# akamiru/bce

Measured on AMD Instinct MI355X. Metric: MB/s compressed, higher is better.
Workload: dtype u8/u32 integer

## Files before the change

### bce_amd/csrc/api.hip

```cpp
#include <condition_variable>
#include <functional>
#include <mutex>
#include <thread>
#include <new>
#include <utility>

#include "bce_cost.h"
#include "common.h"
#include "host_coder.h"
#include "scan_coder.h"

#include <dlfcn.h>
#include <errno.h>
#include <fcntl.h>
#include <sys/file.h>
#include <sys/mman.h>
#include <sys/stat.h>
#include <unistd.h>

using namespace bce;

#ifndef K3_BATCH_MID
#define K3_BATCH_MID 8u
#endif
// ... 336 lines not shown
  bool wide_once = false;
  int dfs_try = 0;
  const uint32_t dfs_enter[2];
  FlushPredictor predict;
  uint32_t round_limit = kNoLimit;
  bool paused = false;

  Enumeration(bce_hip_ctx *ctx, std::function<int(uint64_t)> to)
      : c(ctx), sink(std::move(to)), env(ctx), n(ctx->n), dfs_enter{env.dfs_enter, 2048u} {
    for (int i = 0; i < 8; ++i) { const uint32_t Ci = c->zeros[(i + 7) & 7]; cur_nodes += (Ci && n - Ci) ? 1 : 0; }
  }
  bool finished() const { return ctl.done_round != 0xFFFFFFFFu; }
  int flush() { BCE_TRY(sink(ctl.sym_total)); ctl.sym_total = 0; return BCE_HIP_OK; }
  int grow_lists() { BCE_TRY(k3_grow_lists(c, ctl)); ctl.overflow = 0; return BCE_HIP_OK; }
  int clock_start() { BCE_HIP_TRY(c, hipEventRecord(c->ev0, c->stream)); return BCE_HIP_OK; }
  int clock_stop(bool read_ctl) {
    BCE_HIP_TRY(c, hipEventRecord(c->ev1, c->stream));
    if (read_ctl) BCE_TRY(k3_sync_ctl(c, &ctl));
    else BCE_HIP_TRY(c, hipEventSynchronize(c->ev1));
    float ms = 0;
    if (hipEventElapsedTime(&ms, c->ev0, c->ev1) == hipSuccess) c->stats.k3_ms += ms;
    return BCE_HIP_OK;
  }

  int run() {
    paused = false;
    for (Next next = Next::kRounds; next != Next::kFinished && next != Next::kPaused;) {
      BCE_TRY(gate_regain(c));
      next = Next::kRounds;
      BCE_TRY(pause(&next));
      if (next == Next::kRounds) BCE_TRY(depth_first(&next));
      if (next == Next::kRounds) BCE_TRY(batch(&next));
    }
// ... 46 lines not shown
      while (cut < b.rounds && est < want) { est += nn; nn *= 2; ++cut; }
      b.rounds = cut ? cut : 1u;
    }
    if (!env.no_predict && have_ctl && !ctl.need_flush) b.rounds = predict.rounds_that_fit(b.rounds, c->sym_cap, ctl.sym_total, decaying);
    return b;
  }
  int run_batch(const Batch &b) {
    const uint32_t first = c->round;
    RoctxRange range("bce K3 rounds");
    BCE_TRY(clock_start());
    switch (b.how) {
      case Kernels::kTail: BCE_TRY(k3_tail(c, b.rounds)); break;
      case Kernels::kSmall: BCE_TRY(k3_rounds_small(c, b.rounds, b.nodes, b.growing)); break;
      case Kernels::kWide: BCE_TRY(k3_rounds(c, b.rounds, b.nodes)); break;
    }
    BCE_TRY(clock_stop(true));
    if (ctl.stalled) return k3_stalled(c);
    uint32_t executed = ctl.tail_rounds;
    if (b.how == Kernels::kTail) {
      BCE_TRY(k3_fetch_tail_runs(c, executed));
    } else {
      const bool stopped = ctl.need_flush || ctl.overflow || (b.how == Kernels::kSmall && ctl.small_bail);
      executed = stopped ? ctl.skip_round - first : b.rounds;
      if (executed > b.rounds) return k3_bad_skip(c, ctl, first, b.rounds);
      BCE_TRY(k3_fetch_runs(c, first, executed));
      if (executed) predict.record(reinterpret_cast<const RunEntry *>(c->h_runs), executed, decaying);
    }
    c->round = first + executed;
    return BCE_HIP_OK;
  }
  int batch(Next *next) {
    const Batch b = plan();
    if (!b.rounds) return flush();
    BCE_TRY(run_batch(b));
    if (b.how == Kernels::kSmall && ctl.small_bail) { BCE_TRY(k3_clear_small_bail(c)); wide_once = true; }
    if (ctl.overflow) {
      BCE_TRY(grow_lists());
      have_ctl = true; cur_nodes = 0;
      for (int p = 0; p < 8; ++p) cur_nodes += (uint64_t)ctl.cnt[c->round & 1u][p][0] + ctl.cnt[c->round & 1u][p][1];
      *next = Next::kSameRound;
// ... 124 lines not shown
  (void)hipSetDevice(c->device);
  if (c->coder) c->coder->drain();
  if (c->stream) (void)hipStreamSynchronize(c->stream);
  if (c->k4_stream) (void)hipStreamSynchronize(c->k4_stream);
  if (c->copy_stream) (void)hipStreamSynchronize(c->copy_stream);
  DevBuf *bufs[] = {&c->text, &c->bwt, &c->sa[0], &c->sa[1], &c->key[0], &c->key[1], &c->rank, &c->k2, &c->nrk, &c->act[0], &c->act[1], &c->khi[0], &c->khi[1], &c->dl[0], &c->dl[1], &c->dl[2], &c->dl[3], &c->kflag, &c->actv[0], &c->actv[1],
                    &c->rs_hist, &c->blk, &c->ptmp[0], &c->ptmp[1], &c->gran, &c->nlist[0], &c->nlist[1], &c->ctl, &c->tilecnt,
                    &c->tileoff, &c->runs, &c->smwords, &c->k3tw, &c->k3grp, &c->truns, &c->skey[0], &c->skey[1], &c->sval[0], &c->sval[1], &c->sout,
                    &c->sesc, &c->stat, &c->crc_tab, &c->dcfg, &c->k4w, &c->scanrec, &c->dfs, &c->skey_alt, &c->sesc_alt, &c->rs_hist_k4, &c->cost_acc, &c->cost_runs, &c->cmp_res, &c->hook[0], &c->hook[1], &c->hook[2]};
  for (DevBuf *b : bufs) release(*b);
  for (DevBuf &b : c->qbuf) release(b);
  for (auto &par : c->dlist) for (DevBuf &b : par) release(b);
  k4_prepin_join(c, true);
  if (c->h_ctl) (void)hipHostFree(c->h_ctl);
  if (c->h_small) (void)hipHostFree(c->h_small);
  if (c->h_big) big_host_free(c, c->h_big, c->h_big_cap, c->h_big_registered);
  for (void *q : c->dec_pin) if (q) (void)hipHostFree(q);
  if (c->h_runs) (void)hipHostFree(c->h_runs);
  if (c->h_truns) (void)hipHostFree(c->h_truns);
  if (c->coder) c->coder->drain();
  for (FlushSlot &sl : c->slot) {
    slot_free_host(sl, &c->reg_unmaps);
    if (sl.ev_start) (void)hipEventDestroy(sl.ev_start);
    if (sl.ev_copy) (void)hipEventDestroy(sl.ev_copy);
    if (sl.ev_kend) (void)hipEventDestroy(sl.ev_kend);
    if (sl.h_cost_runs) (void)hipHostFree(sl.h_cost_runs);
  }
  if (c->ev_k4) (void)hipEventDestroy(c->ev_k4);
  if (c->ev_k3_batch) (void)hipEventDestroy(c->ev_k3_batch);
  for (hipEvent_t e : c->ev_k4_done) if (e) (void)hipEventDestroy(e);
// ... 282 lines not shown
  if (c->stat.cap < need || c->dcfg.cap < sizeof(PlaneCfg) * 8) return BCE_HIP_E_STATE;
  BCE_HIP_TRY(c, hipMemcpyAsync(c->dcfg.p, c->cfg, sizeof(PlaneCfg) * 8, hipMemcpyHostToDevice, c->stream));
  BCE_TRY(ensure(c, c->skey[0], (size_t)count * 4));
  BCE_TRY(ensure(c, c->sesc, (size_t)count * 4));
  BCE_HIP_TRY(c, hipMemcpyAsync(c->skey[0].p, key_words, (size_t)count * 4, hipMemcpyHostToDevice, c->stream));
  BCE_HIP_TRY(c, hipMemcpyAsync(c->sesc.p, esc_words, (size_t)count * 4, hipMemcpyHostToDevice, c->stream));
  BCE_HIP_TRY(c, hipStreamSynchronize(c->stream));
  BCE_TRY(k4_flush(c, count, c->slot[0]));
  memcpy(out_records, c->slot[0].h_out, (size_t)count * 8);
  uint32_t nq = 0;
  BCE_TRY(k4_long_runs(c, count, &nq));
  if (long_runs) *long_runs = nq;
  return BCE_HIP_OK;
}

static int encode_start(bce_hip_ctx *c) {
  c->gate_wait_s = 0; c->gate_held_s = 0; c->gate_lent = false;
  gate_acquire(c);
  BCE_HIP_TRY(c, hipSetDevice(c->device));
  const uint32_t n = c->n;
  k4_prepin(c, n);
  BCE_TRY(k4_prepare(c));
  BCE_TRY(k3_begin(c));
  uint32_t C[8];
  for (int i = 0; i < 8; ++i) C[i] = c->zeros[(i + 7) & 7];
  c->coder->begin(c->config, C, n);
  memset(c->plane_syms, 0, sizeof c->plane_syms);
  c->stats.symbols = 0; c->stats.flushes = 0; c->stats.t_model = 0; c->stats.t_model_kernels = 0; c->stats.t_coder = 0;
  return BCE_HIP_OK;
}
static int encode_end(bce_hip_ctx *c, const EnumCtl &ctl, double t_enc0) {
  gate_release(c);
  c->gate_lent = false;
  static const bool gate_timing = getenv("BCE_HIP_GATE_TIMING") != nullptr;
  const double t_gpu_done = now_s();
  {
    const double tw = now_s();
    c->coder->drain();
    c->stats.t_coder += now_s() - tw;
    for (FlushSlot &sl : c->slot) account_slot(c, sl);
  }
  if (c->coder->failed()) { snprintf(c->err, sizeof c->err, "host allocation failed in a range-coder thread"); return BCE_HIP_E_NOMEM; }
  c->stats.t_coder_busy = c->coder->busy_seconds();
// ... 4 lines not shown
  c->stage = 4;
  c->stats.t_enum = c->stats.k3_ms * 1e-3;
  if (gate_timing)
    fprintf(stderr, "gate: ctx %p waited %.1f ms, held %.1f ms of %.1f ms from encode's start to its last flush queued (K3 %.1f ms, model %.1f ms, %llu flushes); coders' tail %.1f ms\n",
            (void *)c, c->gate_wait_s * 1e3, c->gate_held_s * 1e3, (t_gpu_done - t_enc0) * 1e3, c->stats.k3_ms, c->stats.t_model * 1e3,
            (unsigned long long)c->stats.flushes, (now_s() - t_gpu_done) * 1e3);
  return BCE_HIP_OK;
}

static int encode_body(bce_hip_ctx *c);
int bce_hip_encode(bce_hip_ctx *c) { return gate_on_error(c, bce_guarded(c, [&] { return encode_body(c); })); }
static int encode_body(bce_hip_ctx *c) {
  BCE_TRY(check_stage(c, 3));
  PhaseScope phase(c, 3);
  const double t_enc0 = now_s();
  BCE_TRY(encode_start(c));
  Enumeration e(c, [&](uint64_t nsym) { return flush_symbols(c, nsym); });
  BCE_TRY(e.run());
  return encode_end(c, e.ctl, t_enc0);
}

static bool early_enum_applies(const bce_hip_ctx *c) {
  const char *e = getenv("BCE_HIP_EARLY_ENUM");
  return !(e && e[0] == '0' && !e[1]) && k1_two_halves(c);
}
static uint32_t early_round_limit(uint32_t h) {
  uint32_t limit = 8u * h;
  if (const char *e = getenv("BCE_HIP_EARLY_CAP")) { const unsigned long v = strtoul(e, nullptr, 10); if (v < limit) limit = (uint32_t)v; }
  return limit;
}
constexpr uint32_t kEarlyDepthMinN = 1u << 22;
static const uint8_t kEarlyDepth[9] = {0, 0, 0, 0, 0, 9, 0, 0, 0};
static int compress_early_body(bce_hip_ctx *c) {
  BCE_TRY(check_stage(c, 1));
  BCE_HIP_TRY(c, hipSetDevice(c->device));
  c->stage = 1; c->enum_active = false;
  uint32_t h = 0;
  double t0 = now_s();
  PhaseScope phase(c, 1);
  {
    RoctxRange range("bce K1 first sort + provisional BWT");
    BCE_TRY(k1_first_sort(c, &h, c->n >= kEarlyDepthMinN ? kEarlyDepth : nullptr));
    BCE_TRY(k1_provisional_bwt(c));
  }
  double t_bwt = now_s() - t0;
  t0 = now_s();
  phase.set(2);
  {
    RoctxRange range("bce K2 planes + rank directory (provisional)");
    BCE_TRY(k2_build_planes(c));
  }
  double t_planes = now_s() - t0;
  uint32_t zeros0[8];
  memcpy(zeros0, c->zeros, sizeof zeros0);

  phase.set(6);
  const double t_enc0 = now_s();
  BCE_TRY(encode_start(c));
  Enumeration e(c, [&](uint64_t nsym) { return flush_symbols(c, nsym); });
  e.round_limit = early_round_limit(h);
  BCE_TRY(e.run());
  if (!e.paused) { gate_release(c); c->gate_lent = false; }
  const uint32_t paused_at = c->round;
  const uint64_t early_syms = c->stats.symbols;
  const double t_early = now_s() - t_enc0;
  uint64_t early_plane[8];
  memcpy(early_plane, c->plane_syms, sizeof early_plane);

  t0 = now_s();
  {
    RoctxRange range("bce K1 second half + BWT");
    BCE_TRY(k1_finish(c));
    BCE_TRY(k1_final_bwt(c, c->k1_first_final));
  }
  t_bwt += now_s() - t0;
  if (!c->k1_first_final) {
    t0 = now_s();
    RoctxRange range("bce K2 planes + rank directory");
    BCE_TRY(k2_build_planes(c));
    t_planes += now_s() - t0;
    if (memcmp(zeros0, c->zeros, sizeof zeros0) != 0) {
      snprintf(c->err, sizeof c->err, "early rounds: the planes of the provisional and of the final BWT differ in their zero counts");
      return BCE_HIP_E_INTERNAL;
    }
  }
  c->stats.t_bwt = t_bwt;
  c->stats.t_planes = t_planes;
  const double t_second = now_s() - t_enc0 - t_early;
  const uint32_t early_limit = e.round_limit;
  const bool early_paused = e.paused;
// ... 414 lines not shown
```

### bce_amd/csrc/bce_core.h

```cpp
#pragma once
#include <stdint.h>

#if defined(__HIPCC__)
#define BCE_HD __host__ __device__ __forceinline__
#else
#define BCE_HD inline
#endif

namespace bce {

constexpr int kMaxK = 31;
constexpr uint32_t kGranuleBits = 96;

struct Granule { uint32_t cum, w0, w1, w2; };
struct Node { uint32_t s, x0, x1; };

BCE_HD uint32_t popc32(uint32_t x) {
#if defined(__HIP_DEVICE_COMPILE__)
  return (uint32_t)__popc(x);
#else
  return (uint32_t)__builtin_popcount(x);
#endif
}

BCE_HD uint32_t div96(uint32_t s) {
#if defined(__HIP_DEVICE_COMPILE__)
  return __umulhi(s, 0xAAAAAAABu) >> 6;
#else
  return (uint32_t)(((uint64_t)s * 0xAAAAAAABull) >> 38);
#endif
// ... 191 lines not shown
```

### bce_amd/csrc/common.h

```cpp
#pragma once
#include <hip/hip_runtime.h>
#include <stdint.h>
#include <stdio.h>
#include <stdlib.h>
#include <string.h>

#include <atomic>
#include <chrono>
#include <condition_variable>
#include <exception>
#include <new>
#include <memory>
#include <mutex>
#include <thread>
#include <vector>

#include <sys/mman.h>

#include "../../include/bce_hip.h"
#include "bce_core.h"
#include "host_coder.h"

namespace bce {

// ... 61 lines not shown
inline void reg_map_settle(void *q, size_t bytes) { (void)madvise(q, (bytes + 4095) & ~(size_t)4095, MADV_NOHUGEPAGE); }
inline void huge_unmap(void *q, size_t bytes) { if (q) (void)munmap(q, (bytes + 4095) & ~(size_t)4095); }
inline size_t slot_map_bytes(size_t cap) { return (cap * 8 + 16 + 4095) & ~(size_t)4095; }
inline void slot_free_host(FlushSlot &s, uint32_t *unmaps = nullptr) {
  if (s.h_out) {
    if (s.registered) {
      if (s.ev_copy) (void)hipEventSynchronize(s.ev_copy);
      (void)hipHostUnregister(s.h_out);
      huge_unmap(s.h_out, slot_map_bytes(s.cap));
      if (unmaps) ++*unmaps;
    } else (void)hipHostFree(s.h_out);
  }
  s.h_out = nullptr; s.cap = 0; s.registered = false;
}

struct RunEntry { uint64_t start; uint32_t count; uint32_t round; };

namespace qb {
enum Id {
  cnt_res,
  cnt_pat, cnt_off, cnt_out,
  loc_res,
  loc_lo, loc_cnt, loc_drop, loc_start, loc_lin, loc_bsum,
  loc_key0, loc_key1, loc_val0, loc_val1,
  loc_pat, loc_off, loc_hits, loc_pos,
  near_res,
  near_pat, near_off, near_out,
  near_hits, near_pos, near_dist,
  cls_res,
  cls_kind, cls_pat,
// ... 45 lines not shown
  bool gate_held = false;
  bool gate_lent = false;
  double gate_t0 = 0, gate_wait_s = 0, gate_held_s = 0;
  uint32_t flush_seq = 0;
  hipEvent_t copy_busy = nullptr;
  hipEvent_t ev0 = nullptr, ev1 = nullptr, ev_k4 = nullptr;
  char err[256] = {0};

  uint32_t n = 0;
  int stage = 0;
  int phase = 0;
  uint32_t offset = 0;
  uint8_t config[9][32];
  bce::PlaneCfg cfg[8];
  uint32_t zeros[8] = {0};
  bool k1_unique = false;
  bool k1_valid = false;
  int sa_res = 0;
  int k1_res = 0;
  uint32_t k1_h = 0;
  bool k1_first_final = false;
  bool k1_carry = false;
  uint32_t k1_h_asked = 0;
  uint64_t plane_syms[8] = {0};
  uint32_t dbg_dfs_budget = 0, dbg_no_dfs = 0, dbg_no_tail = 0, dbg_no_skip = 0, dbg_no_small = 0, dbg_step_small = 0, dbg_no_fused = 0, dbg_no_local = 0, dbg_capp_div = 0, dbg_local_from = 0, dbg_local_budget = 0, dbg_tail_round = 0;
  uint32_t dbg_dec_budget = 0;
  uint32_t dbg_oom = 0;
  uint64_t sym_cap_user = 0;
  bool sync_flush = false;
  bce_hip_progress_fn progress = nullptr;
// ... 26 lines not shown
  bce::DevBuf scanrec;
  bce::DevBuf stat, dcfg, k4w;
  bce::DevBuf cost_acc, cost_runs;
  bce::DevBuf crc_tab;
  uint32_t crc_tab_grid = 0;
  bce::DevBuf cmp_res;
  bce::DevBuf qbuf[bce::qb::count];
  bce::DevBuf hook[3];
  bool crc_const_ready = false;
  bool text_loaded = false;
  uint32_t stat_off[8] = {0};
  bool model_hook = false;

  void *h_ctl = nullptr, *h_runs = nullptr;
  void *h_small = nullptr;
  void *h_big = nullptr;
  size_t h_big_cap = 0;
  uint32_t dec_restarts = 0;
  uint64_t dec_list_grows = 0, dec_split_rounds = 0;
  uint32_t reg_maps = 0, reg_unmaps = 0;
  bool h_big_registered = false;
  void *dec_pin[3] = {nullptr, nullptr, nullptr};
  size_t dec_pin_cap[3] = {0, 0, 0};
  bce::FlushSlot slot[3];
  int slot_next = 0;

  uint32_t round = 0;
  bool enum_active = false;
  std::vector<bce::RunEntry> run_log[8];

// ... 180 lines not shown
int kd_parse(bce_hip_ctx *c, const uint32_t *d_len, const uint32_t *d_pos, const uint8_t *d_query, uint32_t q, uint32_t min_len, bool sizing,
             uint32_t *d_ops, uint64_t ops_cap, uint8_t *d_lits, uint64_t lits_cap, bce_hip_parse_info *info);
int kd_patch(bce_hip_ctx *c, const uint32_t *d_ops, uint32_t nops, const uint8_t *d_lits, uint64_t nlits, bool sizing, uint8_t *d_out,
             uint64_t cap, uint64_t *out_len);
int kd_nsv(bce_hip_ctx *c, const uint32_t *d_vals, uint32_t n, uint32_t *d_psv, uint32_t *d_nsv);
constexpr uint32_t NSV_TREE_BLOCK = 2048;
int nsv_trees(bce_hip_ctx *c, const uint32_t *vals, uint32_t n, uint32_t *NB_out);
int kd_maxrep(bce_hip_ctx *c, const uint32_t *sa, const uint32_t *d_lcp, uint32_t n, const uint8_t *text, const uint8_t *bw, uint32_t min_len,
              uint32_t max_len, uint32_t order, uint32_t limit, bce_hip_maxrep *d_out, uint8_t *d_bytes, uint32_t bytes_per, bce_hip_maxrep_info *info);
int kd_lpf(bce_hip_ctx *c, const uint32_t *sa, uint32_t max_len, bool mirror, uint32_t *d_lpf, uint32_t *d_src);
int kd_self_mirror(bce_hip_ctx *c, const uint32_t *d_lpf, const uint32_t *d_src, const uint8_t *d_text, uint32_t n);
int kd_self_parse(bce_hip_ctx *c, uint32_t n, uint32_t min_len, bool with_src, bool sizing, uint32_t *d_ops, uint64_t ops_cap, uint8_t *d_lits,
                  uint64_t lits_cap, bce_hip_parse_info *info);
int kd_sa_gather(bce_hip_ctx *c, const uint32_t *sa, const uint32_t *rank, uint32_t n, uint32_t *d_sa, uint32_t *d_isa);
int kd_sufcheck(bce_hip_ctx *c, const uint8_t *d_text, const uint32_t *d_sa, uint32_t n, uint64_t *bad, uint32_t *reason);
int k2_build_planes(bce_hip_ctx *c);
int k2_get_plane_bits(bce_hip_ctx *c, int plane, uint8_t *out);
int k2_rank1(bce_hip_ctx *c, int plane, const uint32_t *idx, uint32_t count, uint32_t *out);
int k3_begin(bce_hip_ctx *c);
int k3_rounds(bce_hip_ctx *c, uint32_t count, uint64_t nodes_hint);
int k3_rounds_small(bce_hip_ctx *c, uint32_t count, uint64_t cur_nodes, bool growing);
int k3_round_masked(bce_hip_ctx *c, uint32_t mask, bool repeat);
int k3_clear_need_flush(bce_hip_ctx *c);
int k3_clear_small_bail(bce_hip_ctx *c);
int k3_dfs_tail(bce_hip_ctx *c, const EnumCtl &ctl, uint32_t enter, bool *done);
int k3_tail(bce_hip_ctx *c, uint32_t max_rounds = K3_TAIL_MAXROUNDS);
int k3_fetch_tail_runs(bce_hip_ctx *c, uint32_t rounds);
int k3_sync_ctl(bce_hip_ctx *c, EnumCtl *out);
int k3_fetch_runs(bce_hip_ctx *c, uint32_t first_round, uint32_t count);
int k3_get_nodes(bce_hip_ctx *c, int plane, uint32_t *out, uint32_t cap, uint32_t *count);
int k3_reset_symbols(bce_hip_ctx *c);
int k3_grow_symbols(bce_hip_ctx *c, uint64_t cap);
int k4_prepare(bce_hip_ctx *c);
int k3_grow_lists(bce_hip_ctx *c, const EnumCtl &ctl);
uint64_t k3_symbol_capacity(const bce_hip_ctx *c, uint32_t n);
void k4_prepin(bce_hip_ctx *c, uint32_t n);
void k4_prepin_join(bce_hip_ctx *c, bool drop);
int k4_flush(bce_hip_ctx *c, uint64_t nsym, FlushSlot &slot);
int k4_flush_async(bce_hip_ctx *c, uint64_t nsym, FlushSlot &slot, bool copy_out = true);
int k4_long_runs(bce_hip_ctx *c, uint64_t nsym, uint32_t *count);
int k4_cost_begin(bce_hip_ctx *c);
int k4_cost_async(bce_hip_ctx *c, uint64_t nsym, FlushSlot &slot);
int k4_cost_end(bce_hip_ctx *c, uint64_t acc[16]);

int radix_sort_pairs(bce_hip_ctx *c, uint32_t *key[2], uint32_t *val[2], uint32_t n, uint32_t first_bit, uint32_t bits, int *res,
                     uint32_t max_digit_bits = 8);
int radix_sort_pairs_on(bce_hip_ctx *c, hipStream_t stream, DevBuf &hist, uint32_t *key[2], uint32_t *val[2], uint32_t n,
                        uint32_t first_bit, uint32_t bits, int *res, uint32_t max_digit_bits = 8);
// ... 6 lines not shown
```

### bce_amd/csrc/k1_bwt.hip

```cpp
#include <stdlib.h>

#include <utility>

#include "common.h"
#include "scan_util.h"

namespace bce {

constexpr int K1_T = 256;

constexpr uint32_t K1_MAXB = 1024;
struct K1Plan { uint32_t nb, per_block; };
static K1Plan k1_plan(uint32_t n) {
  const uint32_t chunk = 2048;
  uint32_t chunks = (uint32_t)(((uint64_t)n + chunk - 1) / chunk);
  if (!chunks) chunks = 1;
  uint32_t nb = chunks < K1_MAXB ? chunks : K1_MAXB;
  uint32_t cpb = (chunks + nb - 1) / nb;
  nb = (chunks + cpb - 1) / cpb;
  return {nb, cpb * chunk};
}

enum K1Word : uint32_t {
  K1W_GROUPS = 0,
// ... 607 lines not shown
static int k1_first_sort_wide(bce_hip_ctx *c, const uint8_t *T, uint32_t n, bool sentinel, const uint8_t *want_by_bits, bool may_carry) {
  const size_t b4 = (size_t)n * 4;
  for (int i = 0; i < 2; ++i) { BCE_TRY(ensure(c, c->sa[i], b4)); BCE_TRY(ensure(c, c->key[i], b4)); BCE_TRY(ensure(c, c->khi[i], b4)); }
  BCE_TRY(ensure(c, c->rank, b4));
  BCE_TRY(ensure(c, c->k2, b4));
  BCE_TRY(ensure(c, c->nrk, b4));
  BCE_TRY(ensure(c, c->kflag, (size_t)n + 16));
  for (int i = 0; i < 2; ++i) { BCE_TRY(ensure(c, c->act[i], b4)); BCE_TRY(ensure(c, c->actv[i], b4)); }
  BCE_TRY(ensure(c, c->blk, (size_t)(K1_MAXB + K1W_END) * 4));
  K1Buffers v(c, n);
  const uint32_t g = v.g;

  const uint32_t nbytes = sentinel ? n - 1u : n;
  BCE_HIP_TRY(c, hipMemsetAsync(v.word(K1W_HIST), 0, 256 * 4, c->stream));
  hipLaunchKernelGGL(k1_bytehist_kernel, dim3(g < 1024u ? g : 1024u), dim3(K1_T), 0, c->stream, T, nbytes, v.word(K1W_HIST));
  uint32_t hist[256];
  BCE_TRY(read_back(c, hist, v.word(K1W_HIST), sizeof hist));
  uint16_t code[256];
  uint32_t sigma = sentinel ? 1u : 0u;
  for (int b = 0; b < 256; ++b) { code[b] = (uint16_t)sigma; if (hist[b]) ++sigma; }
  uint32_t bits = ceil_log2(sigma);
  if (bits < 1) bits = 1;
  uint32_t nsym = 64u / bits;
  if (nsym > 16u) nsym = 16u;
  const uint32_t most = nsym;
  const uint32_t want_h = want_by_bits && bits <= 8u ? want_by_bits[bits] : 0u;
  if (want_h && want_h < nsym) nsym = want_h;
  c->k1_h_asked = nsym;
  if (const char *e = getenv("BCE_K1_KEYBITS")) { const uint32_t kb = (uint32_t)strtoul(e, nullptr, 10); if (kb >= bits) nsym = kb / bits < most ? kb / bits : most; }
  const uint32_t keybits = nsym * bits;
  const char *ce = getenv("BCE_HIP_CARRY_BYTE");
  const bool carry = may_carry && !sentinel && keybits + 8u <= 64u && !(ce && ce[0] == '0' && !ce[1]);
  const uint32_t first_bit = carry ? 8u : 0u;
  {
    if (!c->h_small) BCE_TRY(pin_alloc(c, &c->h_small, 4096));
    memcpy(c->h_small, code, sizeof code);
    BCE_HIP_TRY(c, hipMemcpyAsync(v.word(K1W_CODE), c->h_small, sizeof code, hipMemcpyHostToDevice, c->stream));
  }

  {
    const uint32_t per = K1_T * K1I_E;
    hipLaunchKernelGGL(k1_init64_kernel, dim3((uint32_t)(((uint64_t)n + per - 1) / per)), dim3(K1_T), 0, c->stream, T, n, nbytes,
                       reinterpret_cast<const uint16_t *>(v.word(K1W_CODE)), bits, nsym, carry ? 1u : 0u, v.lo[0], v.hi[0], v.val[0]);
  }
  int res = 0;
  BCE_TRY(radix_sort_wide(c, v.lo, v.hi, v.val, n, first_bit, keybits, &res, 9));
  v.lap("first sort", nsym, n, 0);
  BCE_HIP_TRY(c, hipGetLastError());
  c->k1_res = res;
  c->k1_h = nsym;
  c->k1_carry = carry;
  return BCE_HIP_OK;
}

static int k1_finish_wide(bce_hip_ctx *c, uint32_t n) {
  K1View v(c, n);
  BCE_TRY(v.first_ranks());
  c->k1_first_final = v.m == 0 || v.h >= n;
  while (v.m > 0 && v.h < n) {
    BCE_TRY(v.segmented_round());
    if (v.nd) BCE_TRY(v.sort_deferred());
// ... 124 lines not shown
```

### bce_amd/csrc/k2_planes.hip

```cpp
#include "common.h"
#include "scan_util.h"

namespace bce {

constexpr int K2_T = 256;
constexpr uint32_t K2_CHUNK = 3072;

struct K2Plan { uint32_t chunks, nb, cpb; };
static K2Plan k2_plan(uint32_t n) {
  uint32_t chunks = (uint32_t)(((uint64_t)n + 1 + K2_CHUNK - 1) / K2_CHUNK);
  uint32_t nb = chunks < 1024u ? chunks : 1024u;
  uint32_t cpb = (chunks + nb - 1) / nb;
  nb = (chunks + cpb - 1) / cpb;
  return {chunks, nb, cpb};
}

__device__ __forceinline__ void k2_load12(const uint8_t *__restrict__ B, uint64_t pos0, uint32_t n, uint32_t w[3]) {
  if (pos0 + 12 <= n) {
    const uint32_t *p = reinterpret_cast<const uint32_t *>(B + pos0);
    w[0] = p[0]; w[1] = p[1]; w[2] = p[2];
  } else {
    w[0] = w[1] = w[2] = 0;
    for (uint32_t i = 0; i < 12; ++i)
      if (pos0 + i < n) w[i >> 2] |= (uint32_t)B[pos0 + i] << (8 * (i & 3));
// ... 81 lines not shown
  for (uint64_t p = (uint64_t)blockIdx.x * blockDim.x + threadIdx.x; p < n; p += (uint64_t)gridDim.x * blockDim.x) {
    const uint32_t g = div96((uint32_t)p), o = (uint32_t)p - g * 96u;
    const Granule q = G[g];
    const uint32_t wv = o < 32 ? q.w0 : (o < 64 ? q.w1 : q.w2);
    out[p] = (uint8_t)((wv >> (o & 31u)) & 1u);
  }
}
__global__ void k2_rank_kernel(const Granule *__restrict__ G, const uint32_t *__restrict__ idx, uint32_t cnt,
                               uint32_t *__restrict__ out) {
  for (uint32_t i = blockIdx.x * blockDim.x + threadIdx.x; i < cnt; i += gridDim.x * blockDim.x) {
    const uint32_t s = idx[i], g = div96(s);
    out[i] = granule_rank1(G[g], s - g * 96u);
  }
}

int k2_build_planes(bce_hip_ctx *c) {
  const uint32_t n = c->n;
  const K2Plan pl = k2_plan(n);
  c->ngran = pl.chunks * 32u;
  BCE_TRY(ensure(c, c->gran, (size_t)8 * c->ngran * sizeof(Granule)));
  BCE_TRY(ensure(c, c->ptmp[0], n));
  BCE_TRY(ensure(c, c->ptmp[1], n));
  BCE_TRY(ensure(c, c->blk, (size_t)(pl.nb + 16) * 4));
  uint32_t *zc = c->blk.as<uint32_t>();
  uint32_t *zout = zc + pl.nb;
  const uint8_t *cur = c->bwt.as<uint8_t>();
  for (int j = 0; j < 8; ++j) {
    uint8_t *nxt = j < 7 ? c->ptmp[j & 1].as<uint8_t>() : nullptr;
    Granule *G = c->gran.as<Granule>() + (size_t)j * c->ngran;
    hipLaunchKernelGGL(k2_count_kernel, dim3(pl.nb), dim3(K2_T), 0, c->stream, cur, n, pl.cpb, pl.chunks, j, zc);
    hipLaunchKernelGGL(k2_partition_kernel, dim3(pl.nb), dim3(K2_T), 0, c->stream, cur, nxt, n, pl.cpb, pl.chunks,
                       pl.nb, j, zc, G, zout);
    cur = nxt;
  }
  BCE_TRY(read_back(c, c->zeros, zout, 32));
  BCE_HIP_TRY(c, hipGetLastError());
  return BCE_HIP_OK;
}

int k2_get_plane_bits(bce_hip_ctx *c, int plane, uint8_t *out) {
  const uint32_t n = c->n;
  DevBuf tmp;
  BCE_TRY(ensure(c, tmp, n));
  const Granule *G = c->gran.as<Granule>() + (size_t)plane * c->ngran;
  hipLaunchKernelGGL(k2_bits_kernel, dim3(1024), dim3(256), 0, c->stream, G, n, tmp.as<uint8_t>());
  hipError_t e = hipMemcpyAsync(out, tmp.p, n, hipMemcpyDeviceToHost, c->stream);
  if (e == hipSuccess) e = hipStreamSynchronize(c->stream);
  release(tmp);
  BCE_HIP_TRY(c, e);
  return BCE_HIP_OK;
// ... 25 lines not shown
```

### bce_amd/csrc/k3_enumerate.hip

```cpp
#include <stdlib.h>

#include "common.h"
#include "scan_util.h"
#include "k3_args.h"

namespace bce {

__device__ __forceinline__ void tile_prefix(const K3Args &a, uint32_t tp[9], uint32_t (*cn)[2] = nullptr, uint32_t *skip = nullptr) {
  if (skip) *skip = a.ctl->need_flush | a.ctl->overflow;
  uint32_t acc = 0;
#pragma unroll
  for (int p = 0; p < 8; ++p) {
    tp[p] = acc;
    const uint32_t m0 = a.ctl->cnt[a.par][p][0], m1 = a.ctl->cnt[a.par][p][1];
    if (cn) { cn[p][0] = m0; cn[p][1] = m1; }
    acc += (m0 + m1 + K3_TILE - 1) / K3_TILE;
  }
  tp[8] = acc;
}

__device__ __forceinline__ void group_prefix(const uint32_t tp[9], uint32_t gp[9]) {
  uint32_t acc = 0;
#pragma unroll
  for (int p = 0; p < 8; ++p) { gp[p] = acc; acc += (tp[p + 1] - tp[p] + 255u) >> 8; }
// ... 846 lines not shown
  BCE_TRY(k3_size_tile_arrays(c));
  BCE_HIP_TRY(c, hipMemsetAsync(&c->ctl.as<EnumCtl>()->overflow, 0, sizeof(uint32_t), c->stream));
  return BCE_HIP_OK;
}

uint64_t k3_symbol_capacity(const bce_hip_ctx *c, uint32_t n) {
  uint64_t cap = c->sym_cap_user;
  if (!cap) {
    const char *env = getenv("BCE_HIP_FLUSH_RECORDS");
    const uint64_t want = (uint64_t)8 * n + 1024, soft = env ? strtoull(env, nullptr, 10) : ((uint64_t)1 << 24);
    cap = want < soft ? want : soft;
  }
  return cap;
}

int k3_begin(bce_hip_ctx *c) {
  const uint32_t n = c->n;
  for (int par = 0; par < 2; ++par) {
    c->capL[par] = initial_capP(c, n, full_capP(n), par);
    BCE_TRY(ensure(c, c->nlist[par], (size_t)8 * c->capL[par] * sizeof(Node)));
  }
  c->stats.list_grows = 0; c->stats.list_nodes = c->capL[0] > c->capL[1] ? c->capL[0] : c->capL[1];
  BCE_TRY(k3_size_tile_arrays(c));
  BCE_TRY(ensure(c, c->ctl, sizeof(EnumCtl)));
  BCE_TRY(ensure(c, c->runs, (size_t)K3_MAXBATCH * 8 * sizeof(RunEntry)));
  if (!c->h_ctl) BCE_TRY(pin_alloc(c, &c->h_ctl, sizeof(EnumCtl)));
  if (!c->h_runs) BCE_TRY(pin_alloc(c, &c->h_runs, (size_t)K3_MAXBATCH * 8 * sizeof(RunEntry)));
  const uint64_t cap = k3_symbol_capacity(c, n);
  c->sym_cap = cap;
  BCE_TRY(ensure(c, c->skey[0], (size_t)cap * 4));
  BCE_TRY(ensure(c, c->sesc, (size_t)cap * 4));
  if (c->overlap && !c->scan_mode) {
    BCE_TRY(ensure(c, c->skey_alt, (size_t)cap * 4));
    BCE_TRY(ensure(c, c->sesc_alt, (size_t)cap * 4));
  }
  if (c->scan_mode) BCE_TRY(ensure(c, c->scanrec, (size_t)cap * 4));
  EnumCtl ctl;
  memset(&ctl, 0, sizeof ctl);
  ctl.sym_cap = cap;
  ctl.done_round = 0xFFFFFFFFu;
  for (int i = 0; i < 8; ++i) {
    const uint32_t C = c->zeros[(i + 7) & 7];
    if (C && n - C) {
      Node root = {0u, C, n - C};
      BCE_HIP_TRY(c, hipMemcpyAsync(c->nlist[0].as<Node>() + (size_t)i * c->capL[0], &root, sizeof root,
                                    hipMemcpyHostToDevice, c->stream));
      BCE_HIP_TRY(c, hipStreamSynchronize(c->stream));
      ctl.cnt[0][i][0] = 1;
    }
  }
  BCE_HIP_TRY(c, hipMemcpyAsync(c->ctl.p, &ctl, sizeof ctl, hipMemcpyHostToDevice, c->stream));
  BCE_HIP_TRY(c, hipStreamSynchronize(c->stream));
  BCE_TRY(ensure(c, c->smwords, (size_t)K3_SMALL_MAXTILES * 8));
  BCE_HIP_TRY(c, hipMemsetAsync(c->smwords.p, 0, (size_t)K3_SMALL_MAXTILES * 8, c->stream));
  c->round = 0;
  c->enum_active = true;
  for (int p = 0; p < 8; ++p) c->run_log[p].clear();
  c->stats.k3_ms = 0; c->stats.k3_launches = 0;
  return BCE_HIP_OK;
}

int k3_rounds(bce_hip_ctx *c, uint32_t count, uint64_t nodes_hint) {
  if (count > K3_MAXBATCH) count = K3_MAXBATCH;
  uint64_t want = nodes_hint ? (nodes_hint * 2 + K3_TILE - 1) / K3_TILE + 16 : 2048;
  const uint32_t grid = (uint32_t)(want < 2048 ? want : 2048);
  const bool fused = !c->dbg_no_fused && !k4_in_flight(c);
  if (fused && !c->k3_count2_grid) {
// ... 74 lines not shown
  c->stats.k3_launches += 1.0;
  return BCE_HIP_OK;
}

int k3_fetch_tail_runs(bce_hip_ctx *c, uint32_t rounds) {
  if (!rounds) return BCE_HIP_OK;
  BCE_HIP_TRY(c, hipMemcpyAsync(c->h_truns, c->truns.p, (size_t)rounds * 8 * sizeof(RunEntry), hipMemcpyDeviceToHost, c->stream));
  BCE_HIP_TRY(c, hipStreamSynchronize(c->stream));
  const RunEntry *r = reinterpret_cast<const RunEntry *>(c->h_truns);
  for (uint32_t i = 0; i < rounds; ++i)
    for (int p = 0; p < 8; ++p)
      if (r[(size_t)i * 8 + p].count) c->run_log[p].push_back(r[(size_t)i * 8 + p]);
  return BCE_HIP_OK;
}

int k3_sync_ctl(bce_hip_ctx *c, EnumCtl *out) {
  BCE_HIP_TRY(c, hipMemcpyAsync(c->h_ctl, c->ctl.p, sizeof(EnumCtl), hipMemcpyDeviceToHost, c->stream));
  BCE_HIP_TRY(c, hipStreamSynchronize(c->stream));
  memcpy(out, c->h_ctl, sizeof(EnumCtl));
  return BCE_HIP_OK;
}

int k3_fetch_runs(bce_hip_ctx *c, uint32_t first_round, uint32_t count) {
  (void)first_round;
  if (!count) return BCE_HIP_OK;
  BCE_HIP_TRY(c, hipMemcpyAsync(c->h_runs, c->runs.p, (size_t)count * 8 * sizeof(RunEntry), hipMemcpyDeviceToHost,
                                c->stream));
  BCE_HIP_TRY(c, hipStreamSynchronize(c->stream));
  const RunEntry *r = reinterpret_cast<const RunEntry *>(c->h_runs);
  for (uint32_t i = 0; i < count; ++i)
    for (int p = 0; p < 8; ++p)
      if (r[(size_t)i * 8 + p].count) c->run_log[p].push_back(r[(size_t)i * 8 + p]);
  return BCE_HIP_OK;
}

int k3_reset_symbols(bce_hip_ctx *c) {
  EnumCtl *d = c->ctl.as<EnumCtl>();
  BCE_HIP_TRY(c, hipMemsetAsync(&d->sym_total, 0, sizeof(uint64_t), c->stream));
  BCE_HIP_TRY(c, hipMemsetAsync(&d->need_flush, 0, sizeof(uint32_t), c->stream));
  for (int p = 0; p < 8; ++p) c->run_log[p].clear();
  return BCE_HIP_OK;
}

int k3_grow_symbols(bce_hip_ctx *c, uint64_t cap) {
  if (cap >= (1ull << 31)) return BCE_HIP_E_OVERFLOW;
  BCE_HIP_TRY(c, hipStreamSynchronize(c->stream));
  if (c->k4_stream) BCE_HIP_TRY(c, hipStreamSynchronize(c->k4_stream));
// ... 38 lines not shown
```

### bce_amd/csrc/k4_model.hip

```cpp
#include <algorithm>

#include <stdlib.h>
#include <sys/mman.h>

#include "common.h"
#include "scan_util.h"

namespace bce {

constexpr int K4_T = 256;
constexpr uint32_t K4_LONG = 256;
constexpr uint8_t K4_NOT_LONG = 0xFE;
constexpr uint8_t K4_NO_HALVE = 0xFF;

struct K4Args {
  const uint32_t *keys, *vals;
  uint8_t *stat;
  const PlaneCfg *cfg;
  uint64_t *out;
  const uint32_t *esc;
  uint8_t *histT;
  uint8_t *stateW;
  uint32_t *winfo;
  uint8_t *haltW;
// ... 277 lines not shown
  __shared__ uint32_t cntbuf[K4_T / 64][32];
  const uint32_t lane = threadIdx.x & 63u, w = threadIdx.x >> 6;
  volatile uint32_t *cb = cntbuf[w];
  const uint64_t ltm = (1ull << lane) - 1ull;
  const uint64_t nwaves = (uint64_t)gridDim.x * (K4_T / 64);
  for (uint64_t win = (uint64_t)blockIdx.x * (K4_T / 64) + w; win * 64 < a.nsym; win += nwaves) {
    if (a.haltW[win] == K4_NOT_LONG) continue;
    const uint32_t info = a.winfo[win];
    const uint32_t hkey = a.keys[win * 64];
    const uint32_t k = key_k(hkey);
    uint32_t C = lane < k ? (uint32_t)a.stateW[win * 32 + lane] : 0u;
    (void)k4_replay(a, win * 64, win * 64 + (info & 127u), info >> 7, k, C, cb, lane, ltm);
  }
}

int k4_prepare(bce_hip_ctx *c) {
  uint32_t off = 0;
  for (int p = 0; p < 8; ++p) {
    plane_cfg_init(c->cfg[p], c->config[p]);
    c->stat_off[p] = off;
    off += (c->cfg[p].stat_bytes + 15u) & ~15u;
  }
  BCE_TRY(ensure(c, c->stat, off ? off : 16));
  BCE_TRY(ensure(c, c->dcfg, sizeof(PlaneCfg) * 8));
  BCE_HIP_TRY(c, hipMemsetAsync(c->stat.p, 0, off ? off : 16, c->stream));
  BCE_HIP_TRY(c, hipMemcpyAsync(c->dcfg.p, c->cfg, sizeof(PlaneCfg) * 8, hipMemcpyHostToDevice, c->stream));
  BCE_HIP_TRY(c, hipStreamSynchronize(c->stream));
  return BCE_HIP_OK;
}

struct K4Work { size_t nwin, o_hist, o_state, o_info, o_queue, o_halt, o_bits, o_qc, bytes; };
static K4Work k4_work(uint32_t nsym) {
  K4Work w;
  w.nwin = ((size_t)nsym + 63) / 64;
  auto up16 = [](size_t v) { return (v + 15) & ~(size_t)15; };
  w.o_hist = 0; w.o_state = w.o_hist + w.nwin * 32; w.o_info = w.o_state + w.nwin * 32;
  w.o_queue = up16(w.o_info + w.nwin * 4); w.o_halt = w.o_queue + (w.nwin / 4 + 2) * 8; w.o_bits = up16(w.o_halt + w.nwin);
  w.o_qc = up16(w.o_bits + w.nwin * 8);
  w.bytes = w.o_qc + 16;
  return w;
}

// ... 194 lines not shown
```

Baseline: 926.5.

## Remove host syncs from encode setup and fold run readback into ctl sync

The encoder setup (k4_prepare, k3_begin) now runs earlier, during the early-depth path, and queues work without host synchronisation. The K3 root nodes and control block are initialised by a small device kernel instead of per-plane memcpy+sync. The plane zero counts are copied asynchronously into a pinned block and checked later. Each K3 batch's run entries are fetched together with the control block in one stream sync, removing one round trip per batch. Risks: zero counts computed from the host histogram must match the K2 output (an explicit check covers this), and extra run rows are copied when a batch stops early. An env knob for K1 radix digit bits is also added.

```diff
diff --git a/bce_amd/csrc/api.hip b/bce_amd/csrc/api.hip
--- a/bce_amd/csrc/api.hip
+++ b/bce_amd/csrc/api.hip
@@ -374,9 +374,9 @@
   int flush() { BCE_TRY(sink(ctl.sym_total)); ctl.sym_total = 0; return BCE_HIP_OK; }
   int grow_lists() { BCE_TRY(k3_grow_lists(c, ctl)); ctl.overflow = 0; return BCE_HIP_OK; }
   int clock_start() { BCE_HIP_TRY(c, hipEventRecord(c->ev0, c->stream)); return BCE_HIP_OK; }
-  int clock_stop(bool read_ctl) {
+  int clock_stop(bool read_ctl, uint32_t run_rows = 0) {
     BCE_HIP_TRY(c, hipEventRecord(c->ev1, c->stream));
-    if (read_ctl) BCE_TRY(k3_sync_ctl(c, &ctl));
+    if (read_ctl) BCE_TRY(k3_sync_ctl(c, &ctl, run_rows));
     else BCE_HIP_TRY(c, hipEventSynchronize(c->ev1));
     float ms = 0;
     if (hipEventElapsedTime(&ms, c->ev0, c->ev1) == hipSuccess) c->stats.k3_ms += ms;
@@ -453,7 +453,7 @@
       case Kernels::kSmall: BCE_TRY(k3_rounds_small(c, b.rounds, b.nodes, b.growing)); break;
       case Kernels::kWide: BCE_TRY(k3_rounds(c, b.rounds, b.nodes)); break;
     }
-    BCE_TRY(clock_stop(true));
+    BCE_TRY(clock_stop(true, b.how == Kernels::kTail ? 0u : b.rounds));
     if (ctl.stalled) return k3_stalled(c);
     uint32_t executed = ctl.tail_rounds;
     if (b.how == Kernels::kTail) {
@@ -462,7 +462,7 @@
       const bool stopped = ctl.need_flush || ctl.overflow || (b.how == Kernels::kSmall && ctl.small_bail);
       executed = stopped ? ctl.skip_round - first : b.rounds;
       if (executed > b.rounds) return k3_bad_skip(c, ctl, first, b.rounds);
-      BCE_TRY(k3_fetch_runs(c, first, executed));
+      k3_take_runs(c, executed);
       if (executed) predict.record(reinterpret_cast<const RunEntry *>(c->h_runs), executed, decaying);
     }
     c->round = first + executed;
@@ -617,6 +617,7 @@
   k4_prepin_join(c, true);
   if (c->h_ctl) (void)hipHostFree(c->h_ctl);
   if (c->h_small) (void)hipHostFree(c->h_small);
+  if (c->h_prep) (void)hipHostFree(c->h_prep);
   if (c->h_big) big_host_free(c, c->h_big, c->h_big_cap, c->h_big_registered);
   for (void *q : c->dec_pin) if (q) (void)hipHostFree(q);
   if (c->h_runs) (void)hipHostFree(c->h_runs);
@@ -929,19 +930,24 @@
   return BCE_HIP_OK;
 }
 
-static int encode_start(bce_hip_ctx *c) {
-  c->gate_wait_s = 0; c->gate_held_s = 0; c->gate_lent = false;
-  gate_acquire(c);
+static int encode_prepare(bce_hip_ctx *c, bool wait) {
   BCE_HIP_TRY(c, hipSetDevice(c->device));
   const uint32_t n = c->n;
   k4_prepin(c, n);
-  BCE_TRY(k4_prepare(c));
+  BCE_TRY(k4_prepare(c, false));
   BCE_TRY(k3_begin(c));
   uint32_t C[8];
   for (int i = 0; i < 8; ++i) C[i] = c->zeros[(i + 7) & 7];
   c->coder->begin(c->config, C, n);
   memset(c->plane_syms, 0, sizeof c->plane_syms);
   c->stats.symbols = 0; c->stats.flushes = 0; c->stats.t_model = 0; c->stats.t_model_kernels = 0; c->stats.t_coder = 0;
+  if (wait) BCE_HIP_TRY(c, hipStreamSynchronize(c->stream));
+  return BCE_HIP_OK;
+}
+static int encode_gate(bce_hip_ctx *c) {
+  c->gate_wait_s = 0; c->gate_held_s = 0; c->gate_lent = false;
+  gate_acquire(c);
+  BCE_HIP_TRY(c, hipSetDevice(c->device));
   return BCE_HIP_OK;
 }
 static int encode_end(bce_hip_ctx *c, const EnumCtl &ctl, double t_enc0) {
@@ -976,7 +982,8 @@
   BCE_TRY(check_stage(c, 3));
   PhaseScope phase(c, 3);
   const double t_enc0 = now_s();
-  BCE_TRY(encode_start(c));
+  BCE_TRY(encode_prepare(c, true));
+  BCE_TRY(encode_gate(c));
   Enumeration e(c, [&](uint64_t nsym) { return flush_symbols(c, nsym); });
   BCE_TRY(e.run());
   return encode_end(c, e.ctl, t_enc0);
@@ -1003,22 +1010,23 @@
   {
     RoctxRange range("bce K1 first sort + provisional BWT");
     BCE_TRY(k1_first_sort(c, &h, c->n >= kEarlyDepthMinN ? kEarlyDepth : nullptr));
+    zeros_from_hist(c->k1_hist, c->zeros);
+    phase.set(6);
+    BCE_TRY(encode_prepare(c, false));
     BCE_TRY(k1_provisional_bwt(c));
   }
   double t_bwt = now_s() - t0;
   t0 = now_s();
-  phase.set(2);
   {
     RoctxRange range("bce K2 planes + rank directory (provisional)");
-    BCE_TRY(k2_build_planes(c));
+    BCE_TRY(k2_build_planes(c, c->h_prep->zout));
   }
   double t_planes = now_s() - t0;
   uint32_t zeros0[8];
   memcpy(zeros0, c->zeros, sizeof zeros0);
 
-  phase.set(6);
   const double t_enc0 = now_s();
-  BCE_TRY(encode_start(c));
+  BCE_TRY(encode_gate(c));
   Enumeration e(c, [&](uint64_t nsym) { return flush_symbols(c, nsym); });
   e.round_limit = early_round_limit(h);
   BCE_TRY(e.run());
@@ -1036,6 +1044,10 @@
     BCE_TRY(k1_final_bwt(c, c->k1_first_final));
   }
   t_bwt += now_s() - t0;
+  if (memcmp(zeros0, c->h_prep->zout, sizeof zeros0) != 0) {
+    snprintf(c->err, sizeof c->err, "early rounds: the planes of the provisional and of the final BWT differ in their zero counts");
+    return BCE_HIP_E_INTERNAL;
+  }
   if (!c->k1_first_final) {
     t0 = now_s();
     RoctxRange range("bce K2 planes + rank directory");
diff --git a/bce_amd/csrc/bce_core.h b/bce_amd/csrc/bce_core.h
--- a/bce_amd/csrc/bce_core.h
+++ b/bce_amd/csrc/bce_core.h
@@ -14,6 +14,13 @@
 
 struct Granule { uint32_t cum, w0, w1, w2; };
 struct Node { uint32_t s, x0, x1; };
+
+inline void zeros_from_hist(const uint32_t hist[256], uint32_t zeros[8]) {
+  for (int j = 0; j < 8; ++j) zeros[j] = 0;
+  for (uint32_t b = 0; b < 256; ++b)
+    for (int j = 0; j < 8; ++j)
+      if (!((b >> j) & 1u)) zeros[j] += hist[b];
+}
 
 BCE_HD uint32_t popc32(uint32_t x) {
 #if defined(__HIP_DEVICE_COMPILE__)
diff --git a/bce_amd/csrc/common.h b/bce_amd/csrc/common.h
--- a/bce_amd/csrc/common.h
+++ b/bce_amd/csrc/common.h
@@ -99,6 +99,7 @@
   s.h_out = nullptr; s.cap = 0; s.registered = false;
 }
 
+struct PrepBlock { PlaneCfg cfg[8]; uint32_t zout[8]; };
 struct RunEntry { uint64_t start; uint32_t count; uint32_t round; };
 
 namespace qb {
@@ -174,6 +175,7 @@
   uint8_t config[9][32];
   bce::PlaneCfg cfg[8];
   uint32_t zeros[8] = {0};
+  uint32_t k1_hist[256] = {0};
   bool k1_unique = false;
   bool k1_valid = false;
   int sa_res = 0;
@@ -230,6 +232,7 @@
 
   void *h_ctl = nullptr, *h_runs = nullptr;
   void *h_small = nullptr;
+  bce::PrepBlock *h_prep = nullptr;
   void *h_big = nullptr;
   size_t h_big_cap = 0;
   uint32_t dec_restarts = 0;
@@ -440,7 +443,7 @@
                   uint64_t lits_cap, bce_hip_parse_info *info);
 int kd_sa_gather(bce_hip_ctx *c, const uint32_t *sa, const uint32_t *rank, uint32_t n, uint32_t *d_sa, uint32_t *d_isa);
 int kd_sufcheck(bce_hip_ctx *c, const uint8_t *d_text, const uint32_t *d_sa, uint32_t n, uint64_t *bad, uint32_t *reason);
-int k2_build_planes(bce_hip_ctx *c);
+int k2_build_planes(bce_hip_ctx *c, uint32_t *pinned_zout = nullptr);
 int k2_get_plane_bits(bce_hip_ctx *c, int plane, uint8_t *out);
 int k2_rank1(bce_hip_ctx *c, int plane, const uint32_t *idx, uint32_t count, uint32_t *out);
 int k3_begin(bce_hip_ctx *c);
@@ -452,12 +455,13 @@
 int k3_dfs_tail(bce_hip_ctx *c, const EnumCtl &ctl, uint32_t enter, bool *done);
 int k3_tail(bce_hip_ctx *c, uint32_t max_rounds = K3_TAIL_MAXROUNDS);
 int k3_fetch_tail_runs(bce_hip_ctx *c, uint32_t rounds);
-int k3_sync_ctl(bce_hip_ctx *c, EnumCtl *out);
+int k3_sync_ctl(bce_hip_ctx *c, EnumCtl *out, uint32_t run_rows = 0);
+void k3_take_runs(bce_hip_ctx *c, uint32_t count);
 int k3_fetch_runs(bce_hip_ctx *c, uint32_t first_round, uint32_t count);
 int k3_get_nodes(bce_hip_ctx *c, int plane, uint32_t *out, uint32_t cap, uint32_t *count);
 int k3_reset_symbols(bce_hip_ctx *c);
 int k3_grow_symbols(bce_hip_ctx *c, uint64_t cap);
-int k4_prepare(bce_hip_ctx *c);
+int k4_prepare(bce_hip_ctx *c, bool wait = true);
 int k3_grow_lists(bce_hip_ctx *c, const EnumCtl &ctl);
 uint64_t k3_symbol_capacity(const bce_hip_ctx *c, uint32_t n);
 void k4_prepin(bce_hip_ctx *c, uint32_t n);
diff --git a/bce_amd/csrc/k1_bwt.hip b/bce_amd/csrc/k1_bwt.hip
--- a/bce_amd/csrc/k1_bwt.hip
+++ b/bce_amd/csrc/k1_bwt.hip
@@ -645,8 +645,8 @@
   const uint32_t nbytes = sentinel ? n - 1u : n;
   BCE_HIP_TRY(c, hipMemsetAsync(v.word(K1W_HIST), 0, 256 * 4, c->stream));
   hipLaunchKernelGGL(k1_bytehist_kernel, dim3(g < 1024u ? g : 1024u), dim3(K1_T), 0, c->stream, T, nbytes, v.word(K1W_HIST));
-  uint32_t hist[256];
-  BCE_TRY(read_back(c, hist, v.word(K1W_HIST), sizeof hist));
+  uint32_t *const hist = c->k1_hist;
+  BCE_TRY(read_back(c, hist, v.word(K1W_HIST), sizeof c->k1_hist));
   uint16_t code[256];
   uint32_t sigma = sentinel ? 1u : 0u;
   for (int b = 0; b < 256; ++b) { code[b] = (uint16_t)sigma; if (hist[b]) ++sigma; }
@@ -675,7 +675,9 @@
                        reinterpret_cast<const uint16_t *>(v.word(K1W_CODE)), bits, nsym, carry ? 1u : 0u, v.lo[0], v.hi[0], v.val[0]);
   }
   int res = 0;
-  BCE_TRY(radix_sort_wide(c, v.lo, v.hi, v.val, n, first_bit, keybits, &res, 9));
+  uint32_t digit = 9;
+  if (const char *e = getenv("BCE_K1_DIGITBITS")) { const uint32_t d = (uint32_t)strtoul(e, nullptr, 10); if (d >= 8 && d <= 10) digit = d; }
+  BCE_TRY(radix_sort_wide(c, v.lo, v.hi, v.val, n, first_bit, keybits, &res, digit));
   v.lap("first sort", nsym, n, 0);
   BCE_HIP_TRY(c, hipGetLastError());
   c->k1_res = res;
diff --git a/bce_amd/csrc/k2_planes.hip b/bce_amd/csrc/k2_planes.hip
--- a/bce_amd/csrc/k2_planes.hip
+++ b/bce_amd/csrc/k2_planes.hip
@@ -119,7 +119,7 @@
   }
 }
 
-int k2_build_planes(bce_hip_ctx *c) {
+int k2_build_planes(bce_hip_ctx *c, uint32_t *pinned_zout) {
   const uint32_t n = c->n;
   const K2Plan pl = k2_plan(n);
   c->ngran = pl.chunks * 32u;
@@ -138,7 +138,8 @@
                        pl.nb, j, zc, G, zout);
     cur = nxt;
   }
-  BCE_TRY(read_back(c, c->zeros, zout, 32));
+  if (pinned_zout) BCE_HIP_TRY(c, hipMemcpyAsync(pinned_zout, zout, 32, hipMemcpyDeviceToHost, c->stream));
+  else BCE_TRY(read_back(c, c->zeros, zout, 32));
   BCE_HIP_TRY(c, hipGetLastError());
   return BCE_HIP_OK;
 }
diff --git a/bce_amd/csrc/k3_enumerate.hip b/bce_amd/csrc/k3_enumerate.hip
--- a/bce_amd/csrc/k3_enumerate.hip
+++ b/bce_amd/csrc/k3_enumerate.hip
@@ -884,6 +884,22 @@
   return cap;
 }
 
+struct K3Roots { uint32_t C[8]; };
+__global__ void k3_init_kernel(EnumCtl *__restrict__ ctl, Node *__restrict__ lists, uint32_t capL, K3Roots roots, uint32_t n, uint64_t sym_cap) {
+  uint32_t *w = reinterpret_cast<uint32_t *>(ctl);
+  for (uint32_t i = threadIdx.x; i < sizeof(EnumCtl) / 4; i += blockDim.x) w[i] = 0;
+  __syncthreads();
+  if (threadIdx.x < 8) {
+    const uint32_t i = threadIdx.x, C = roots.C[i];
+    if (C && n - C) {
+      lists[(size_t)i * capL] = Node{0u, C, n - C};
+      ctl->cnt[0][i][0] = 1;
+    }
+  }
+  if (threadIdx.x == 0) { ctl->sym_cap = sym_cap; ctl->done_round = 0xFFFFFFFFu; }
+}
+static_assert(sizeof(EnumCtl) % 4 == 0, "k3_init_kernel clears the control block word by word");
+
 int k3_begin(bce_hip_ctx *c) {
   const uint32_t n = c->n;
   for (int par = 0; par < 2; ++par) {
@@ -905,22 +921,10 @@
     BCE_TRY(ensure(c, c->sesc_alt, (size_t)cap * 4));
   }
   if (c->scan_mode) BCE_TRY(ensure(c, c->scanrec, (size_t)cap * 4));
-  EnumCtl ctl;
-  memset(&ctl, 0, sizeof ctl);
-  ctl.sym_cap = cap;
-  ctl.done_round = 0xFFFFFFFFu;
-  for (int i = 0; i < 8; ++i) {
-    const uint32_t C = c->zeros[(i + 7) & 7];
-    if (C && n - C) {
-      Node root = {0u, C, n - C};
-      BCE_HIP_TRY(c, hipMemcpyAsync(c->nlist[0].as<Node>() + (size_t)i * c->capL[0], &root, sizeof root,
-                                    hipMemcpyHostToDevice, c->stream));
-      BCE_HIP_TRY(c, hipStreamSynchronize(c->stream));
-      ctl.cnt[0][i][0] = 1;
-    }
-  }
-  BCE_HIP_TRY(c, hipMemcpyAsync(c->ctl.p, &ctl, sizeof ctl, hipMemcpyHostToDevice, c->stream));
-  BCE_HIP_TRY(c, hipStreamSynchronize(c->stream));
+  K3Roots roots;
+  for (int i = 0; i < 8; ++i) roots.C[i] = c->zeros[(i + 7) & 7];
+  hipLaunchKernelGGL(k3_init_kernel, dim3(1), dim3(64), 0, c->stream, c->ctl.as<EnumCtl>(), c->nlist[0].as<Node>(), c->capL[0], roots, n, cap);
+  BCE_HIP_TRY(c, hipGetLastError());
   BCE_TRY(ensure(c, c->smwords, (size_t)K3_SMALL_MAXTILES * 8));
   BCE_HIP_TRY(c, hipMemsetAsync(c->smwords.p, 0, (size_t)K3_SMALL_MAXTILES * 8, c->stream));
   c->round = 0;
@@ -1025,11 +1029,20 @@
   return BCE_HIP_OK;
 }
 
-int k3_sync_ctl(bce_hip_ctx *c, EnumCtl *out) {
+int k3_sync_ctl(bce_hip_ctx *c, EnumCtl *out, uint32_t run_rows) {
+  if (run_rows > K3_MAXBATCH) run_rows = K3_MAXBATCH;
+  if (run_rows) BCE_HIP_TRY(c, hipMemcpyAsync(c->h_runs, c->runs.p, (size_t)run_rows * 8 * sizeof(RunEntry), hipMemcpyDeviceToHost, c->stream));
   BCE_HIP_TRY(c, hipMemcpyAsync(c->h_ctl, c->ctl.p, sizeof(EnumCtl), hipMemcpyDeviceToHost, c->stream));
   BCE_HIP_TRY(c, hipStreamSynchronize(c->stream));
   memcpy(out, c->h_ctl, sizeof(EnumCtl));
   return BCE_HIP_OK;
+}
+
+void k3_take_runs(bce_hip_ctx *c, uint32_t count) {
+  const RunEntry *r = reinterpret_cast<const RunEntry *>(c->h_runs);
+  for (uint32_t i = 0; i < count; ++i)
+    for (int p = 0; p < 8; ++p)
+      if (r[(size_t)i * 8 + p].count) c->run_log[p].push_back(r[(size_t)i * 8 + p]);
 }
 
 int k3_fetch_runs(bce_hip_ctx *c, uint32_t first_round, uint32_t count) {
@@ -1038,10 +1051,7 @@
   BCE_HIP_TRY(c, hipMemcpyAsync(c->h_runs, c->runs.p, (size_t)count * 8 * sizeof(RunEntry), hipMemcpyDeviceToHost,
                                 c->stream));
   BCE_HIP_TRY(c, hipStreamSynchronize(c->stream));
-  const RunEntry *r = reinterpret_cast<const RunEntry *>(c->h_runs);
-  for (uint32_t i = 0; i < count; ++i)
-    for (int p = 0; p < 8; ++p)
-      if (r[(size_t)i * 8 + p].count) c->run_log[p].push_back(r[(size_t)i * 8 + p]);
+  k3_take_runs(c, count);
   return BCE_HIP_OK;
 }
 
diff --git a/bce_amd/csrc/k4_model.hip b/bce_amd/csrc/k4_model.hip
--- a/bce_amd/csrc/k4_model.hip
+++ b/bce_amd/csrc/k4_model.hip
@@ -315,7 +315,8 @@
   }
 }
 
-int k4_prepare(bce_hip_ctx *c) {
+int k4_prepare(bce_hip_ctx *c, bool wait) {
+  if (!c->h_prep) BCE_TRY(pin_alloc(c, reinterpret_cast<void **>(&c->h_prep), sizeof(PrepBlock)));
   uint32_t off = 0;
   for (int p = 0; p < 8; ++p) {
     plane_cfg_init(c->cfg[p], c->config[p]);
@@ -325,8 +326,9 @@
   BCE_TRY(ensure(c, c->stat, off ? off : 16));
   BCE_TRY(ensure(c, c->dcfg, sizeof(PlaneCfg) * 8));
   BCE_HIP_TRY(c, hipMemsetAsync(c->stat.p, 0, off ? off : 16, c->stream));
-  BCE_HIP_TRY(c, hipMemcpyAsync(c->dcfg.p, c->cfg, sizeof(PlaneCfg) * 8, hipMemcpyHostToDevice, c->stream));
-  BCE_HIP_TRY(c, hipStreamSynchronize(c->stream));
+  memcpy(c->h_prep->cfg, c->cfg, sizeof(PlaneCfg) * 8);
+  BCE_HIP_TRY(c, hipMemcpyAsync(c->dcfg.p, c->h_prep->cfg, sizeof(PlaneCfg) * 8, hipMemcpyHostToDevice, c->stream));
+  if (wait) BCE_HIP_TRY(c, hipStreamSynchronize(c->stream));
   return BCE_HIP_OK;
 }
 
```

After: 926.9, median of 2. About the same (+0.0%).
